# KyleJHarper/tyche

Measured on AMD Instinct MI355X. Metric: GiB/s device-resident LZ4 compress+decompress, 1M×16KiB pages, 1/2/4/8 GPU, higher is better.
Workload: dtype u8

## Files before the change

### tyche_amd/csrc/lz4_decode_lc.hip

```cpp
#include <hip/hip_runtime.h>

#include "engine.h"
#include "lane_ring.h"
#include "lds_io.h"
#include "lds_qword.h"

namespace tyche {

#if defined(TYCHE_ABLATE) && TYCHE_ABLATE
#define LC_ABLATE(bit) ((TYCHE_ABLATE & (bit)) != 0)
#else
#define LC_ABLATE(bit) false
#endif

#ifdef TYCHE_PROFILE
__device__ unsigned long long g_lcprof[16];
#define LPROF_DECL                                  \
    unsigned long long _pt = clock64(), _acc[16]; \
    for (int _k = 0; _k < 16; _k++) _acc[_k] = 0;
#define LPROF_MARK(k)                  \
    do {                               \
        unsigned long long _n = clock64(); \
        _acc[k] += _n - _pt;           \
        _pt = _n;                      \
    } while (0)
#define LPROF_ADD(k, v) do { _acc[k] += (unsigned long long)(v); } while (0)
#define LPROF_END                                                              \
    do {                                                                       \
        if (lane == 0)                                                         \
            for (int _k = 0; _k < 16; _k++) atomicAdd(&g_lcprof[_k], _acc[_k]); \
    } while (0)
#else
#define LPROF_DECL
#define LPROF_MARK(k) do { } while (0)
#define LPROF_ADD(k, v) do { } while (0)
#define LPROF_END do { } while (0)
#endif

namespace {

__device__ __forceinline__ void lc_lut_load(const uint32_t *lut, int32_t c, uint32_t *ent) {
    const uint8_t *p = (const uint8_t *)lut + 48 * c;
    const uint64_t a = lq(p), b = lq(p + 8), x = lq(p + 16), y = lq(p + 24);
    ent[0] = (uint32_t)a;
    ent[1] = (uint32_t)(a >> 32);
    ent[2] = (uint32_t)b;
    ent[3] = (uint32_t)(b >> 32);
    ent[4] = (uint32_t)x;
    ent[5] = (uint32_t)(x >> 32);
    ent[6] = (uint32_t)y;
    ent[7] = (uint32_t)(y >> 32);
    ent[8] = ld32(p + 32);
}

#include "lz4_lc_core.h"

template <int32_t R>
struct LCL {
    static_assert(lc_ring_ok<R>(), "ring too small for the flush granule (lc_budget)");
    static constexpr uint32_t win = 0;
    static constexpr uint32_t ring = 64u * kLWS;
    static constexpr uint32_t tab_out = ring + 64u * (uint32_t)R;
    static constexpr uint32_t tab_fl = tab_out + 64u * 8u;
    static constexpr int32_t max_pieces = (lc_budget<R>() + kLcLine - 1) / 16 + 1;
    static constexpr uint32_t own = tab_fl + 64u * 4u;
    static constexpr uint32_t lut = own + ((64u * (uint32_t)max_pieces * 2u + 15u) & ~15u);
    static constexpr uint32_t total = lut + (uint32_t)kLutBytes;
};

struct LMeta {
    const uint8_t *in;
    uint8_t *out;
    uint32_t L, C;
};
__device__ __forceinline__ LMeta lmeta(const tyche_batch_t &b, size_t idx) {
    const PageRef r = batch_page(b, idx);
    return LMeta{r.src, r.dst, r.src_len, r.dst_cap};
}

struct LWin {
    u128 c0, c1, c2, c3;
    uint32_t sh;
};
__device__ __forceinline__ LWin wload(const uint8_t *__restrict__ in, int32_t ns, int32_t L) {
    LWin w;
    if (L >= 16) {
        const int32_t top = L - 16;
        const int32_t a0 = min(ns, top), a1 = min(ns + 16, top), a2 = min(ns + 32, top), a3 = min(ns + 48, top);
        w.c0 = ld16(in + a0);
        w.c1 = ld16(in + a1);
        w.c2 = ld16(in + a2);
        w.c3 = ld16(in + a3);
        w.sh = (uint32_t)min(ns - a0, 16) | ((uint32_t)min(ns + 16 - a1, 16) << 8) |
               ((uint32_t)min(ns + 32 - a2, 16) << 16) | ((uint32_t)min(ns + 48 - a3, 16) << 24);
    } else {
        w.c0 = chunk16z(in, ns, L);
        w.c1 = chunk16z(in, ns + 16, L);
        w.c2 = chunk16z(in, ns + 32, L);
        w.c3 = chunk16z(in, ns + 48, L);
        w.sh = 0;
    }
    return w;
}
__device__ __forceinline__ u128 wshift(u128 v, uint32_t k) {
    k &= 0xFFu;
    return k >= 16u ? (u128)0 : (k == 0u ? v : v >> (8u * k));
}
__device__ __forceinline__ void lc_put_piece(uint8_t *base, int32_t k, u128 v) {
    lq(LC_Q(base, k), (uint64_t)v);
    lq(LC_Q(base, k + 1), (uint64_t)(v >> 64));
}
__device__ __forceinline__ u128 lc_get_piece(const uint8_t *base, int32_t k) {
    return (u128)lq(LC_Q(base, k)) | ((u128)lq(LC_Q(base, k + 1)) << 64);
}
__device__ __forceinline__ void wstore(uint8_t *w16, const LWin &w) {
    if (w.sh == 0) {
        lc_put_piece(w16, 0, w.c0);
        lc_put_piece(w16, 2, w.c1);
        lc_put_piece(w16, 4, w.c2);
        lc_put_piece(w16, 6, w.c3);
    } else {
        lc_put_piece(w16, 0, wshift(w.c0, w.sh));
        lc_put_piece(w16, 2, wshift(w.c1, w.sh >> 8));
        lc_put_piece(w16, 4, wshift(w.c2, w.sh >> 16));
        lc_put_piece(w16, 6, wshift(w.c3, w.sh >> 24));
    }
}

constexpr int kVmDrain = 0x0F70;

__device__ bool lpage_start(const tyche_batch_t &b, uint32_t in_cap, uint32_t out_cap, size_t idx, size_t G,
                            LPage &P, uint8_t *w16) {
    for (; idx < b.count; idx += G) {
        const LMeta m = lmeta(b, idx);
        int32_t rv;
        if (m.L > in_cap || m.C > out_cap) {
            rv = kResultTooLarge;
        } else if (m.C == 0) {
            rv = (m.L == 1 && ld1(m.in) == 0) ? 0 : -1;
        } else if (m.L == 0) {
            rv = -1;
        } else {
            P.in = m.in;
            P.out = m.out;
            P.L = (int32_t)m.L;
            P.C = (int32_t)m.C;
            P.idx = idx;
            P.ip = P.op = P.fl = P.wb = 0;
            P.tail = 0;
            P.lp = P.lrem = P.moff = P.mrem = P.mtok = P.hdr = P.term = 0;
            wstore(w16, wload(P.in, 0, P.L));
            __builtin_amdgcn_s_waitcnt(kVmDrain);
            return true;
        }
        b.results[idx] = rv;
    }
    return false;
}

__device__ __attribute__((aligned(64))) uint8_t g_lc_pad[64];

template <int32_t N>
__device__ __forceinline__ void far_load(const LPage &P, bool far, int32_t src, uint32_t rec, u32x4 (&fv)[N], int32_t t) {
    if (LC_ABLATE(1024)) far = false;
    if (far) {
        const uint8_t *a = P.out + src;
        asm volatile("global_load_dwordx4 %0, %1, off" : "+v"(fv[kFarPer * t]) : "v"(a) : "memory");
        if (kFarPer == 2 && ((rec >> 10) & 63u) > 16u)
            asm volatile("global_load_dwordx4 %0, %1, off offset:16" : "+v"(fv[kFarPer * t + (kFarPer - 1)]) : "v"(a) : "memory");
    }
}
template <int32_t N>
__device__ __forceinline__ void lc_far_wait(u32x4 (&fv)[N]) {
    asm volatile("s_waitcnt vmcnt(4)" ::: "memory");
#pragma unroll
    for (int32_t i = 0; i < N; i++) asm volatile("" : "+v"(fv[i]));
}

#ifndef LC_WPE
#define LC_WPE 2
#endif
template <int32_t R>
__global__ __launch_bounds__(64) __attribute__((amdgpu_waves_per_eu(LC_WPE))) void lz4_decode_lc_kernel(tyche_batch_t b, uint32_t in_cap, uint32_t out_cap) {
    typedef LCL<R> Lay;
    extern __shared__ __attribute__((aligned(16))) uint8_t smem[];
    const uint32_t lane = threadIdx.x;
    uint8_t *ring = smem + Lay::ring + lane * 8u;
    uint8_t *w16 = smem + Lay::win + lane * 8u;
    uint64_t *tab_out = (uint64_t *)(smem + Lay::tab_out);
    uint32_t *tab_fl = (uint32_t *)(smem + Lay::tab_fl);
    uint16_t *own = (uint16_t *)(smem + Lay::own);
    const uint32_t *lut = (const uint32_t *)(smem + Lay::lut);
    const size_t G = (size_t)gridDim.x * 64u;
    if (lane <= 16) {
        uint32_t ent[kLutStride];
        lc_lut_entry((int32_t)lane, ent);
        for (int32_t j = 0; j < kLutStride; j++) ld32(smem + Lay::lut + 48u * lane + 4u * (uint32_t)j, ent[j]);
    }

    LPage P;
    bool live = lpage_start(b, in_cap, out_cap, (size_t)blockIdx.x * 64u + lane, G, P, w16);
    LPROF_DECL
    while (__builtin_amdgcn_ballot_w64(live) != 0) {
        LPROF_ADD(0, 1);
        LPROF_MARK(9);
        const int32_t op0 = P.op;
        int32_t st = live ? kLParse : kLCut, rv = 0, nrec = 0;
        uint32_t rec[kLC + 1];
        u32x4 fv[kFarPer * (kLC + 1)];
#pragma unroll
        for (int32_t i = 0; i < kFarPer * (kLC + 1); i++) fv[i] = u32x4{0u, 0u, 0u, 0u};
        bool go = live, gen = false;
        int32_t need_gen = 0;
        uint64_t wq[4];
        lc_wread(w16, lc_x0(P), wq);
        bool far0 = false, far1 = false;
        int32_t src0 = 0, src1 = 0;
#pragma unroll
        for (int32_t t = 0; t < kLC; t++) {
            rec[t] = 0;
            bool far = false;
            int32_t src = 0;
            if (go) {
                const int32_t k = parse_fast<R>(P, w16, op0, rec[t], far, src, wq);
                if (k == 1) {
                    nrec = t + 1;
                } else {
                    go = false;
                    need_gen = (k == 2 || t == 0) ? 1 : 0;
                    if (k == 0 && t != 0) st = kLCut;
                }
            }
            if (t == 0) {
                far0 = far;
                src0 = src;
            } else if (t == 1) {
                far1 = far;
                src1 = src;
                LPROF_MARK(1);
                __builtin_amdgcn_s_waitcnt(kVmDrain);
                LPROF_MARK(2);
                asm volatile("" ::: "memory");
                far_load(P, far0, src0, rec[0], fv, 0);
                far_load(P, far1, src1, rec[1], fv, 1);
            } else {
                far_load(P, far, src, rec[t], fv, t);
            }
        }
        LPROF_MARK(3);
        rec[kLC] = 0;
        {
            bool far = false;
            int32_t src = 0;
            if (__builtin_amdgcn_ballot_w64(need_gen != 0) != 0 && need_gen)
                gen = parse_slot<R>(P, w16, op0, false, st, rv, rec[kLC], far, src);
            const bool deep = need_gen && !gen && nrec == 0 && st == kLCut;
            if (__builtin_amdgcn_ballot_w64(deep) != 0 && deep) {
                st = kLParse;
                gen = parse_slot<R>(P, w16, op0, true, st, rv, rec[kLC], far, src);
            }
            far_load(P, far && gen, src, rec[kLC], fv, kLC);
        }
        LPROF_MARK(4);
        LPROF_ADD(12, __builtin_amdgcn_ballot_w64(need_gen != 0) != 0);
        const bool ended = live && st == kLEnd;
        const int32_t nwb = (P.lrem > 0 ? P.lp : P.ip) & ~15;
        const bool wlive = live && !ended;
        const LWin nw = wload(wlive ? P.in : g_lc_pad, wlive ? nwb : 0, wlive ? P.L : 64);
        if (ended && rv < 0) {
            nrec = 0;
            gen = false;
        }

        LPROF_MARK(5);
        lc_far_wait(fv);
        if (LC_ABLATE(8192)) {
            const LWin xw = wload(wlive ? P.in : g_lc_pad, wlive ? min(nwb + 64, max(P.L - 64, 0)) : 0, wlive ? P.L : 64);
            __builtin_amdgcn_s_waitcnt(kVmDrain);
            if (xw.c0 == (u128)0x123457 && xw.c3 == (u128)1) P.tail ^= 1;
        }
        if (live && !LC_ABLATE(4096)) {
            u128 farv[kFarPer * (kLC + 1)];
#pragma unroll
            for (int32_t i = 0; i < kFarPer * (kLC + 1); i++) farv[i] = __builtin_bit_cast(u128, fv[i]);
            uint64_t tail = P.tail;
            copy_records<R>(ring, w16, op0, tail, rec, farv, nrec, gen, lut);
            P.tail = tail;
        }
        LPROF_MARK(6);

        if (live && !ended) {
            P.wb = nwb;
            wstore(w16, nw);
        }
        LPROF_MARK(7);
        const int32_t lend = !live ? 0 : (ended && rv < 0) ? P.fl : (P.op & ~(kLcLine - 1));
        const int32_t nl = live ? (lend - P.fl) >> 4 : 0;
        const int32_t incl = wave_incl_sum(nl);
        const int32_t total = (int32_t)rdlane((uint32_t)incl, 63);
        if (total > 0) {
            constexpr int32_t MP = Lay::max_pieces;
            tab_out[lane] = (uint64_t)(uintptr_t)P.out;
            tab_fl[lane] = (uint32_t)P.fl;
#pragma unroll
            for (int32_t k = 0; k < MP; k++)
                if (k < nl) own[incl - nl + k] = (uint16_t)(lane | ((uint32_t)k << 6));
            asm volatile("" ::: "memory");
            const int32_t iters = (total + 63) >> 6;
            uint32_t e[MP];
#pragma unroll
            for (int32_t it = 0; it < MP; it++) e[it] = it < iters ? (uint32_t)own[lane + 64 * it] : 0u;
            uint64_t o[MP];
            int32_t f[MP];
#pragma unroll
            for (int32_t it = 0; it < MP; it++) {
                o[it] = 0;
                f[it] = 0;
                if (it < iters) {
                    const uint32_t L2 = e[it] & 63u;
                    o[it] = tab_out[L2];
                    f[it] = (int32_t)tab_fl[L2] + 16 * (int32_t)(e[it] >> 6);
                }
            }
            u128 v[MP];
#pragma unroll
            for (int32_t it = 0; it < MP; it++)
                v[it] = it < iters ? lc_get_piece(smem + Lay::ring + (e[it] & 63u) * 8u, lc_row<R>(f[it] >> 3))
                                   : (u128)0;
#pragma unroll
            for (int32_t it = 0; it < MP; it++) {
                if ((int32_t)lane + 64 * it < total) {
                    uint8_t *dst = (uint8_t *)(uintptr_t)o[it] + f[it];
                    if (!LC_ABLATE(2048)) st16f(dst, v[it]);
                    else if (v[it] == (u128)0x1234567) dst[0] = 1;
                }
            }
            asm volatile("" ::: "memory");
        }
        if (live) P.fl = lend > P.fl ? lend : P.fl;
        LPROF_MARK(8);
        LPROF_ADD(13, total);
        LPROF_ADD(14, __builtin_popcountll(__builtin_amdgcn_ballot_w64(ended)));

        if (ended) {
            if (rv >= 0) {
                for (int32_t a = P.fl; a < P.op; a += 16) {
                    const u128 v = lc_get_piece(ring, lc_row<R>(a >> 3));
                    if (a + 16 <= P.op) {
                        st16(P.out + a, v);
                    } else {
                        for (int32_t x = a; x < P.op; x++) st1(P.out + x, (uint32_t)(v >> (8 * (x - a))) & 0xFFu);
                    }
                }
            }
            b.results[P.idx] = rv;
            live = lpage_start(b, in_cap, out_cap, P.idx + G, G, P, w16);
        }
        LPROF_MARK(10);
        asm volatile("" ::: "memory");
    }
    LPROF_END;
}

}

#ifdef TYCHE_PROFILE
extern "C" int tyche_debug_lc_profile(unsigned long long *host16, int reset) {
    if (reset) {
        unsigned long long z[16] = {0};
        return hipMemcpyToSymbol(HIP_SYMBOL(g_lcprof), z, sizeof(z)) == hipSuccess ? 0 : 1;
    }
    return hipMemcpyFromSymbol(host16, HIP_SYMBOL(g_lcprof), sizeof(unsigned long long) * 16) == hipSuccess ? 0 : 1;
}
#endif

hipError_t launch_lz4_decode_lc(const tyche_batch_t &b, uint32_t in_cap, uint32_t out_cap, hipStream_t s) {
    if (b.count == 0) return hipSuccess;
    const long r = knob("LZ4_LC_RING", 192);
#if LC_LINE == 16
    const void *k = r == 256   ? (const void *)lz4_decode_lc_kernel<256>
                    : r == 192 ? (const void *)lz4_decode_lc_kernel<192>
                    : r == 160 ? (const void *)lz4_decode_lc_kernel<160>
                               : (const void *)lz4_decode_lc_kernel<128>;
    const size_t lds = r == 256   ? LCL<256>::total
                       : r == 192 ? LCL<192>::total
                       : r == 160 ? LCL<160>::total
                                  : LCL<128>::total;
#else
    const void *k = r == 256 ? (const void *)lz4_decode_lc_kernel<256> : (const void *)lz4_decode_lc_kernel<192>;
    const size_t lds = r == 256 ? LCL<256>::total : LCL<192>::total;
#endif
    const size_t ncu = prepare_launch(k);
    size_t waves = blocks_per_cu(k, 64, lds);
    const long env_waves = knob("LZ4_LC_WAVES", 8);
    if (env_waves > 0) waves = std::min<size_t>(waves, (size_t)env_waves);
    const size_t grid = std::min<size_t>((b.count + 63) / 64, ncu * waves);
    void *args[] = {(void *)&b, &in_cap, &out_cap};
    (void)hipLaunchKernel(k, dim3((unsigned)grid), dim3(64), args, lds, s);
    return hipGetLastError();
}

}
```

### tyche_amd/csrc/lz4_lc_core.h

```cpp
#pragma once

#ifndef LC_FN
#define LC_FN __device__ __forceinline__
#endif
#ifndef LC_RCP
#define LC_RCP(x) __builtin_amdgcn_rcpf(x)
#endif
#ifndef LC_BARRIER
#define LC_BARRIER() asm volatile("" ::: "memory")
#endif
#ifndef LC_Q
#define LC_Q(base, k) ((base) + ((uint32_t)(k) << 9))
#endif
#ifndef LC_PERM
#define LC_PERM(hi, lo, sel) __builtin_amdgcn_perm((hi), (lo), (sel))
#endif
#ifndef LC_UMUL24
#define LC_UMUL24(a, b) __umul24((a), (b))
#define LC_MUL24(a, b) __mul24((a), (b))
#endif

constexpr int32_t kLutStride = 12;
constexpr int32_t kLutBytes = 17 * kLutStride * 4;
LC_FN void lc_lut_entry(int32_t c, uint32_t *ent) {
// ... 82 lines not shown
    lq(LC_Q(ring, r1), o1);
    lq(LC_Q(ring, r2), o2);
    const uint32_t k = (s + (uint32_t)n) >> 3;
    return k == 0 ? o0 : (k == 1 ? o1 : o2);
}

struct LPage {
    const uint8_t *in;
    uint8_t *out;
    int32_t L, C;
    size_t idx;
    int32_t ip;
    int32_t op;
    int32_t fl;
    int32_t wb;
    uint64_t tail;
    int32_t lp, lrem;
    int32_t moff, mrem;
    int32_t mtok;
    int32_t hdr, term;
};

enum : int32_t { kLParse = 0, kLCut = 1, kLEnd = 2 };

#ifndef LC_LINE
#define LC_LINE 16
#endif
constexpr int32_t kLcLine = LC_LINE;
static_assert(kLcLine == 16 || kLcLine == 64, "flush granule");
template <int32_t R>
constexpr int32_t lc_near() { return R - 24; }
template <int32_t R>
constexpr int32_t lc_budget() { return R - 24 - kLcLine; }
template <int32_t R>
constexpr bool lc_ring_ok() { return lc_budget<R>() >= 47; }

LC_FN uint32_t lc_rec(int32_t lpr, int32_t n1, int32_t n2, int32_t off) {
    return (uint32_t)lpr | ((uint32_t)n1 << 6) | ((uint32_t)n2 << 10) | ((uint32_t)off << 16);
}

LC_FN uint64_t win8(uint64_t q0, uint64_t q1, uint64_t q2, uint64_t q3, uint32_t r) {
    const uint32_t k = r >> 3;
    const uint64_t a = k == 0 ? q0 : (k == 1 ? q1 : q2), b = k == 0 ? q1 : (k == 1 ? q2 : q3);
    return funnel8(a, b, r & 7u);
}

LC_FN void lc_wread(const uint8_t *w16, int32_t x, uint64_t (&q)[4]) {
    const int32_t k = x >> 3;
    q[0] = lq(LC_Q(w16, k));
    q[1] = lq(LC_Q(w16, k + 1));
    q[2] = lq(LC_Q(w16, k + 2));
    q[3] = lq(LC_Q(w16, k + 3));
}
LC_FN int32_t lc_x0(const LPage &P) {
    return (P.lrem == 0 && P.mrem == 0 && P.hdr == 0) ? min(P.ip - P.wb, kLW) : 0;
}

template <int32_t R>
LC_FN int32_t parse_fast(LPage &P, const uint8_t *w16, int32_t op0, uint32_t &rec, bool &far, int32_t &src,
                         uint64_t (&q)[4]) {
    const int32_t room = op0 + lc_budget<R>() - P.op;
    const bool isA = (P.mrem != 0) & (P.lrem == 0);
    const int32_t nA = min(P.mrem, 32);
    const int32_t nB = min(min(P.lrem, 15), P.wb + kLW - P.lp);
    const bool isB = (P.lrem != 0) & (nB < P.lrem);
    const bool fresh = (P.lrem == 0) & (P.mrem == 0) & (P.hdr == 0);
    const int32_t x = fresh ? P.ip - P.wb : 0;
    const uint64_t q0 = q[0], q1 = q[1], q2 = q[2], q3 = q[3];
    const uint32_t s = (uint32_t)x & 7u;
    const uint32_t token = (uint32_t)(win8(q0, q1, q2, q3, s) & 0xFFu);
    const int32_t lit = (int32_t)(token >> 4), mn = (int32_t)(token & 15u);
    const int32_t need = 1 + lit + (mn == 15 ? 3 : 2);
    lc_wread(w16, min(fresh ? x + need : P.ip - P.wb, kLW), q);
    const uint64_t h = win8(q0, q1, q2, q3, s + 1u + (uint32_t)(lit & 15));
    const int32_t off = (int32_t)(h & 0xFFFFu), ext = (int32_t)((h >> 16) & 0xFFu);
    const int32_t ml = mn == 15 ? 19 + ext : mn + kMinMatch;
    const bool fitC = x + need <= kLW;
    const bool okC = (lit != 15) & !((mn == 15) & (ext == 255)) &
                     (P.op + lit <= P.C - kMfLimit) & (P.ip + 1 + lit <= P.L - 8) &
                     (off <= P.op + lit) &
                     !((mn == 15) & (P.ip + need > P.L - kLastLiterals)) &
                     (P.op + lit + ml <= P.C - kLastLiterals) &
                     (ml <= 32);
    const int32_t moff = isA ? P.moff : off;
    const int32_t n1 = isA ? 0 : (isB ? nB : lit);
    const int32_t n2f = isA ? nA : (isB ? 0 : ml);
    const int32_t n2 = (LC_FAR16 && moff > lc_near<R>()) ? min(n2f, 16) : n2f;
    const bool fits = n1 + n2 <= room;
    const bool cont = isA | isB;
    const bool stop = !cont & (((P.lrem != 0) & (nB <= 0)) | (fresh & !fitC));
    const bool fast = cont | (fresh & okC);
    const int32_t k = stop ? 0 : (fast ? (fits ? 1 : 0) : 2);
    const bool emit = (k == 1);
    far = emit & (n2 > 0) & (moff > lc_near<R>());
    src = emit ? P.op + n1 - moff : src;
    rec = emit ? lc_rec(n1 > 0 ? (isB ? P.lp - P.wb : x + 1) : 0, n1, n2, moff) : rec;
    P.op += emit ? n1 + n2 : 0;
    P.mrem -= (emit & isA) ? n2 : 0;
    P.lp += (emit & isB) ? n1 : 0;
    P.lrem -= (emit & isB) ? n1 : 0;
    P.ip += (emit & fresh) ? need : 0;
    if (LC_FAR16) {
        P.mrem += (emit & fresh) ? ml - n2 : 0;
        P.moff = (emit & fresh) ? off : P.moff;
    }
    return k;
}


LC_FN uint32_t lbyte(const LPage &P, const uint8_t *w16, int32_t p, bool deep, bool &miss) {
    if (p < P.wb + kLW) {
        const int32_t i = p - P.wb;
        return lb(LC_Q(w16, i >> 3) + (i & 7));
    }
    if (deep) return sbyte(P.in, p, P.L);
    miss = true;
    return 0;
}

template <int32_t R>
LC_FN bool parse_slot(LPage &P, const uint8_t *w16, int32_t op0, bool deep, int32_t &st,
                                           int32_t &rv, uint32_t &rec, bool &far, int32_t &src) {
    constexpr int32_t kBudget = lc_budget<R>();
    const int32_t wend = P.wb + kLW;
    bool miss = false;
    if (P.lrem == 0 && P.mrem == 0 && P.hdr == 0) {
        const int32_t ip = P.ip;
        const uint32_t token = lbyte(P, w16, ip, deep, miss);
        int32_t lit = (int32_t)(token >> 4), pos = 1;
        if (lit == kRunMask) {
            uint32_t s;
            do {
                s = lbyte(P, w16, ip + pos, deep, miss);
                pos++;
                lit += (int32_t)s;
            } while (!miss && ip + pos < P.L - kRunMask && s == 255);
        }
        if (miss) {
            st = kLCut;
            return false;
        }
        const bool last = P.op + lit > P.C - kMfLimit || ip + pos + lit > P.L - 8;
        if (last && (ip + pos + lit != P.L || P.op + lit > P.C)) {
            rv = -(ip + pos) - 1;
            st = kLEnd;
            return false;
        }
        P.term = last ? 1 : 0;
        P.hdr = last ? 0 : 1;
        P.mtok = (int32_t)(token & 15u);
        P.lp = ip + pos;
        P.lrem = lit;
        P.ip = ip + pos + lit;
    }
    int32_t n1 = min(P.lrem, 15);
    n1 = min(n1, wend - P.lp);
    if (n1 < 0) n1 = 0;
    if (P.lrem > 0 && n1 == 0) {
// ... 115 lines not shown
```

### tyche_amd/_build.py

```python
from __future__ import annotations

import concurrent.futures as cf
import os
import subprocess

HERE = os.path.dirname(os.path.abspath(__file__))
CSRC = os.path.join(HERE, "csrc")
BUILD = os.path.join(HERE, "..", "build", "tyche_amd")
LIB = os.path.join(HERE, "libtyche_codec.so")
SOURCES = ["engine.hip", "lz4_decode.hip", "lz4_decode_lane.hip", "lz4_decode_lc.hip", "lz4_encode.hip", "lz4_encode_exact.hip", "lz4_encode_hc.hip", "lz4_encode_large.hip", "lz4_decode_large.hip", "lz4_encode_dict.hip", "lz4_decode_dict.hip", "lz4_dict_train.hip", "zlib_inflate.hip", "zstd_decode.hip", "zstd_encode.hip", "zlib_deflate.hip", "pagegen.hip", "pack.hip", "host_batch.hip",
           "errno_guard.hip"]
HIPCC = os.environ.get("HIPCC", "/opt/rocm/bin/hipcc")
ARCH = "gfx950"
FLAGS = ["--offload-arch=" + ARCH, "-O3", "-fPIC", "-std=c++17", "-Wall", "-Wno-unused-variable",
         "-munsafe-fp-atomics", "-I" + os.path.join(HERE, "..", "include")]
LEGACY_SOURCES = ["legacy/lz4_decode_lane_legacy.hip", "legacy/lz4_decode_quad.hip"]
NO_LSV = ["-mllvm", "-amdgpu-load-store-vectorizer=false"]
SOURCE_FLAGS = {"lz4_encode.hip": NO_LSV, "lz4_encode_dict.hip": NO_LSV, "zstd_encode.hip": NO_LSV, "zlib_deflate.hip": NO_LSV, "zstd_decode.hip": NO_LSV}


def kernel_sources_digest() -> str:
    import hashlib
    h = hashlib.sha256()
    files = sorted(f for f in os.listdir(CSRC) if f.endswith((".hip", ".h")))
    for f in files:
        h.update(f.encode())
        h.update(open(os.path.join(CSRC, f), "rb").read())
    h.update(open(os.path.join(HERE, "..", "include", "tyche_codec.h"), "rb").read())
    return h.hexdigest()[:16]


def _newer(target: str, deps: list[str]) -> bool:
    if not os.path.exists(target):
        return False
    t = os.path.getmtime(target)
    return all(os.path.getmtime(d) <= t for d in deps)


def build(force: bool = False, verbose: bool = False, profile: bool = False, ablate: int = 0,
          eablate: int = 0, defines: tuple = (), legacy: bool = False) -> str:
    if legacy:
        defines = tuple(defines) + ("TYCHE_LEGACY_DECODERS",)
    tag = ("_prof" if profile else "") + (f"_abl{ablate}" if ablate else "") + (f"_eabl{eablate}" if eablate else "") + \
        "".join("_" + d.replace("TYCHE_", "").replace("=", "").lower() for d in defines)
    build_dir = BUILD + tag
    lib_path = LIB.replace(".so", tag + ".so")
    flags = FLAGS + (["-DTYCHE_PROFILE"] if profile else []) + ([f"-DTYCHE_ABLATE={ablate}"] if ablate else []) + \
        ([f"-DTYCHE_EABLATE={eablate}"] if eablate else []) + ["-D" + d for d in defines]
    os.makedirs(build_dir, exist_ok=True)
    headers = [os.path.join(CSRC, f) for f in os.listdir(CSRC) if f.endswith(".h")]
    headers.append(os.path.join(HERE, "..", "include", "tyche_codec.h"))
    objs = []
    jobs = []
    sources = SOURCES[:-1] + (LEGACY_SOURCES if legacy else []) + SOURCES[-1:]
    for src in sources:
        s = os.path.join(CSRC, src)
        o = os.path.join(build_dir, src.replace("/", "_").replace(".hip", ".o"))
        objs.append(o)
        if force or not _newer(o, [s] + headers):
            jobs.append([HIPCC] + flags + SOURCE_FLAGS.get(src, []) + ["-c", s, "-o", o])

    def run(cmd):
        if verbose:
# ... 38 lines not shown
```

### tyche_amd/csrc/engine.h

```cpp
#pragma once
#include <hip/hip_runtime.h>

#include <algorithm>
#include <stdint.h>

#include "../../include/tyche_codec.h"

namespace tyche {

constexpr int32_t kResultTooLarge = INT32_MIN;

constexpr int kMinMatch = 4;
constexpr int kLastLiterals = 5;
constexpr int kMfLimit = 12;
constexpr int kRunMask = 15;

__host__ __device__ inline uint32_t lz4_bound(uint32_t n) {
    return n > 0x7E000000u ? 0u : n + n / 255u + 16u;
}

struct PageRef {
    const uint8_t *src;
    uint32_t src_len;
    uint8_t *dst;
    uint32_t dst_cap;
};

template <typename T>
__device__ __forceinline__ T ld_meta(const T *p, size_t i) {
    return ((const __attribute__((address_space(4))) T *)(uintptr_t)p)[i];
}

__device__ inline PageRef batch_page(const tyche_batch_t &b, size_t i) {
    PageRef r;
    uint64_t so = b.src_offsets ? ld_meta(b.src_offsets, i) : (uint64_t)i * b.src_stride;
    uint64_t dof = b.dst_offsets ? ld_meta(b.dst_offsets, i) : (uint64_t)i * b.dst_stride;
    r.src = (const uint8_t *)b.src + so;
    r.src_len = b.src_lengths ? ld_meta(b.src_lengths, i) : b.src_length;
    r.dst = (uint8_t *)b.dst + dof;
    r.dst_cap = b.dst_capacities ? ld_meta(b.dst_capacities, i) : b.dst_capacity;
    return r;
}

#define WAVE_SYNC() __builtin_amdgcn_wave_barrier()

size_t blocks_per_cu(const void *kernel, uint32_t threads, size_t lds);
size_t page_grid(const void *kernel, uint32_t threads, size_t lds, size_t count, const char *cap_knob = nullptr);

hipError_t launch_lz4_decode(const tyche_batch_t &b, uint32_t in_cap, uint32_t out_cap, hipStream_t s,
                             bool allow_lane = true);
bool lz4_lane_decode_wanted(size_t count, uint32_t in_cap, uint32_t out_cap);
hipError_t launch_lz4_decode_lane(const tyche_batch_t &b, uint32_t in_cap, uint32_t out_cap, hipStream_t s);
hipError_t launch_lz4_decode_quad(const tyche_batch_t &b, uint32_t in_cap, uint32_t out_cap, hipStream_t s);
hipError_t launch_lz4_decode_lc(const tyche_batch_t &b, uint32_t in_cap, uint32_t out_cap, hipStream_t s);
hipError_t launch_lz4_encode(const tyche_batch_t &b, uint32_t in_cap, hipStream_t s);
hipError_t launch_lz4_encode_exact(const tyche_batch_t &b, uint32_t in_cap, hipStream_t s);
hipError_t launch_lz4_encode_hc(const tyche_batch_t &b, uint32_t in_cap, hipStream_t s);
hipError_t launch_lz4_encode_large(const tyche_batch_t &b, uint32_t in_cap, uint32_t min_len, hipStream_t s);
hipError_t launch_lz4_decode_large(const tyche_batch_t &b, uint32_t in_cap, uint32_t out_cap, hipStream_t s);
struct Lz4DictDev {
    const uint8_t *dec;
    const uint16_t *table;
    const uint8_t *enc;
    uint32_t dlen, dpad, enc_len, enc_stride;
};
hipError_t launch_lz4_encode_dict(const tyche_batch_t &b, uint32_t in_cap, const Lz4DictDev &d, bool per_page,
                                  hipStream_t s);
hipError_t launch_lz4_decode_dict(const tyche_batch_t &b, uint32_t in_cap, uint32_t out_cap, const Lz4DictDev &d,
                                  bool per_page, hipStream_t s);
struct TrainResult {
    uint32_t dict_len = 0;
    bool too_long = false;
    uint64_t total_bytes = 0;
    const char *step = "";
};
hipError_t train_lz4_dict(const tyche_batch_t &b, uint32_t in_cap, uint32_t dict_len, hipStream_t s, uint8_t *dict_out,
                          TrainResult *res);
hipError_t launch_pack(const tyche_pack_t &p, hipStream_t s, const char **step);
uint64_t pack_plan_host(size_t n, const int32_t *results, uint32_t max_length, uint32_t align, uint64_t capacity,
                        uint64_t state[2], uint64_t *offsets, uint32_t *lengths);
hipError_t launch_zstd_encode(const tyche_batch_t &b, uint32_t in_cap, hipStream_t s);
hipError_t launch_zlib_deflate(const tyche_batch_t &b, uint32_t in_cap, hipStream_t s);
hipError_t launch_zlib_inflate(const tyche_batch_t &b, uint32_t out_cap, hipStream_t s);
hipError_t launch_zstd_decode(const tyche_batch_t &b, uint32_t in_cap, uint32_t out_cap, hipStream_t s);
size_t zstd_dict_seed_bytes();
void zstd_dict_seed_table(const uint8_t *tail, uint32_t n, void *table_out);
hipError_t launch_zstd_encode_dict(const tyche_batch_t &b, uint32_t in_cap, const Lz4DictDev &d, const void *seed,
                                   bool per_page, hipStream_t s);
hipError_t launch_zstd_decode_dict(const tyche_batch_t &b, uint32_t in_cap, uint32_t out_cap, const Lz4DictDev &d,
                                   bool per_page, hipStream_t s);
class WorkCounter {
  public:
    explicit WorkCounter(hipStream_t s, bool claims = true);
    ~WorkCounter();
    WorkCounter(const WorkCounter &) = delete;
    WorkCounter &operator=(const WorkCounter &) = delete;
    unsigned *get() const { return p_; }

  private:
    hipStream_t s_;
    int dev_ = -1, idx_ = -1;
    unsigned *p_ = nullptr;
};
class ScratchLease {
  public:
    ScratchLease(hipStream_t s, size_t bytes);
    ~ScratchLease();
// ... 23 lines not shown
```

Measured before the change: 191.5.

## Widen LZ4 fast-parse path and alias flush tables over window rows

Result: no change. 192.8, median of 6 (+0.7%).

```diff
diff --git a/tyche_amd/csrc/lz4_decode_lc.hip b/tyche_amd/csrc/lz4_decode_lc.hip
--- a/tyche_amd/csrc/lz4_decode_lc.hip
+++ b/tyche_amd/csrc/lz4_decode_lc.hip
@@ -55,16 +55,23 @@
 
 #include "lz4_lc_core.h"
 
+#ifndef LC_ALIAS
+#define LC_ALIAS 1
+#endif
+
 template <int32_t R>
 struct LCL {
     static_assert(lc_ring_ok<R>(), "ring too small for the flush granule (lc_budget)");
     static constexpr uint32_t win = 0;
     static constexpr uint32_t ring = 64u * kLWS;
-    static constexpr uint32_t tab_out = ring + 64u * (uint32_t)R;
+    static constexpr uint32_t ring_end = ring + 64u * (uint32_t)R;
+    static constexpr uint32_t tab_out = LC_ALIAS ? win : ring_end;
     static constexpr uint32_t tab_fl = tab_out + 64u * 8u;
     static constexpr int32_t max_pieces = (lc_budget<R>() + kLcLine - 1) / 16 + 1;
     static constexpr uint32_t own = tab_fl + 64u * 4u;
-    static constexpr uint32_t lut = own + ((64u * (uint32_t)max_pieces * 2u + 15u) & ~15u);
+    static constexpr uint32_t tab_end = own + ((64u * (uint32_t)max_pieces * 2u + 15u) & ~15u);
+    static_assert(!LC_ALIAS || tab_end <= ring, "the flush tables must fit the window rows they lie over");
+    static constexpr uint32_t lut = LC_ALIAS ? ring_end : tab_end;
     static constexpr uint32_t total = lut + (uint32_t)kLutBytes;
 };
 
@@ -289,10 +296,23 @@
         }
         LPROF_MARK(6);
 
+#if LC_ALIAS
+        u128 np0 = nw.c0, np1 = nw.c1, np2 = nw.c2, np3 = nw.c3;
+        if (nw.sh != 0) {
+            np0 = wshift(np0, nw.sh);
+            np1 = wshift(np1, nw.sh >> 8);
+            np2 = wshift(np2, nw.sh >> 16);
+            np3 = wshift(np3, nw.sh >> 24);
+        }
+        u32x4 nq0 = __builtin_bit_cast(u32x4, np0), nq1 = __builtin_bit_cast(u32x4, np1),
+              nq2 = __builtin_bit_cast(u32x4, np2), nq3 = __builtin_bit_cast(u32x4, np3);
+        asm volatile("" : "+v"(nq0), "+v"(nq1), "+v"(nq2), "+v"(nq3));
+#else
         if (live && !ended) {
             P.wb = nwb;
             wstore(w16, nw);
         }
+#endif
         LPROF_MARK(7);
         const int32_t lend = !live ? 0 : (ended && rv < 0) ? P.fl : (P.op & ~(kLcLine - 1));
         const int32_t nl = live ? (lend - P.fl) >> 4 : 0;
@@ -338,6 +358,16 @@
             asm volatile("" ::: "memory");
         }
         if (live) P.fl = lend > P.fl ? lend : P.fl;
+#if LC_ALIAS
+        asm volatile("" : "+v"(nq0), "+v"(nq1), "+v"(nq2), "+v"(nq3));
+        if (live && !ended) {
+            P.wb = nwb;
+            lc_put_piece(w16, 0, __builtin_bit_cast(u128, nq0));
+            lc_put_piece(w16, 2, __builtin_bit_cast(u128, nq1));
+            lc_put_piece(w16, 4, __builtin_bit_cast(u128, nq2));
+            lc_put_piece(w16, 6, __builtin_bit_cast(u128, nq3));
+        }
+#endif
         LPROF_MARK(8);
         LPROF_ADD(13, total);
         LPROF_ADD(14, __builtin_popcountll(__builtin_amdgcn_ballot_w64(ended)));
diff --git a/tyche_amd/csrc/lz4_lc_core.h b/tyche_amd/csrc/lz4_lc_core.h
--- a/tyche_amd/csrc/lz4_lc_core.h
+++ b/tyche_amd/csrc/lz4_lc_core.h
@@ -158,58 +158,78 @@
     q[2] = lq(LC_Q(w16, k + 2));
     q[3] = lq(LC_Q(w16, k + 3));
 }
-LC_FN int32_t lc_x0(const LPage &P) {
-    return (P.lrem == 0 && P.mrem == 0 && P.hdr == 0) ? min(P.ip - P.wb, kLW) : 0;
-}
+LC_FN int32_t lc_x0(const LPage &P) { return min(P.ip - P.wb, kLW); }
+
+#ifndef LC_STAT
+#define LC_STAT(i, c) do { } while (0)
+#endif
+
+#ifndef LC_FASTX
+#define LC_FASTX 1
+#endif
+constexpr bool kFxM = (LC_FASTX & 1) != 0, kFxL = (LC_FASTX & 2) != 0, kFxH = (LC_FASTX & 4) != 0;
 
 template <int32_t R>
 LC_FN int32_t parse_fast(LPage &P, const uint8_t *w16, int32_t op0, uint32_t &rec, bool &far, int32_t &src,
                          uint64_t (&q)[4]) {
     const int32_t room = op0 + lc_budget<R>() - P.op;
-    const bool isA = (P.mrem != 0) & (P.lrem == 0);
-    const int32_t nA = min(P.mrem, 32);
+    const bool inrun = P.lrem != 0;
+    const bool isA = (P.mrem != 0) & !inrun;
     const int32_t nB = min(min(P.lrem, 15), P.wb + kLW - P.lp);
-    const bool isB = (P.lrem != 0) & (nB < P.lrem);
-    const bool fresh = (P.lrem == 0) & (P.mrem == 0) & (P.hdr == 0);
-    const int32_t x = fresh ? P.ip - P.wb : 0;
+    const bool isB = inrun & (nB < P.lrem) & (nB > 0);
+    const bool isH = kFxH & (P.hdr != 0) & (nB == P.lrem);
+    const bool fresh = !inrun & (P.mrem == 0) & (P.hdr == 0);
+    const int32_t x = P.ip - P.wb;
     const uint64_t q0 = q[0], q1 = q[1], q2 = q[2], q3 = q[3];
     const uint32_t s = (uint32_t)x & 7u;
-    const uint32_t token = (uint32_t)(win8(q0, q1, q2, q3, s) & 0xFFu);
-    const int32_t lit = (int32_t)(token >> 4), mn = (int32_t)(token & 15u);
-    const int32_t need = 1 + lit + (mn == 15 ? 3 : 2);
-    lc_wread(w16, min(fresh ? x + need : P.ip - P.wb, kLW), q);
-    const uint64_t h = win8(q0, q1, q2, q3, s + 1u + (uint32_t)(lit & 15));
+    const uint64_t w0 = win8(q0, q1, q2, q3, s);
+    const uint32_t token = (uint32_t)w0 & 0xFFu;
+    const int32_t lit4 = (int32_t)(token >> 4), lext = (int32_t)((uint32_t)(w0 >> 8) & 0xFFu);
+    const bool isL = kFxL & fresh & (lit4 == 15);
+    const int32_t lit = (kFxL && lit4 == 15) ? 15 + lext : lit4;
+    const int32_t mn = (kFxH && !fresh) ? P.mtok : (int32_t)(token & 15u);
+    const int32_t hl = mn == 15 ? 3 : 2;
+    const int32_t need = fresh ? (isL ? 2 + lit : 1 + lit4 + hl) : (isH ? hl : 0);
+    lc_wread(w16, min(x + need, kLW), q);
+    const uint64_t h = win8(q0, q1, q2, q3, (kFxH && !fresh) ? s : s + 1u + (uint32_t)lit4);
     const int32_t off = (int32_t)(h & 0xFFFFu), ext = (int32_t)((h >> 16) & 0xFFu);
     const int32_t ml = mn == 15 ? 19 + ext : mn + kMinMatch;
-    const bool fitC = x + need <= kLW;
-    const bool okC = (lit != 15) & !((mn == 15) & (ext == 255)) &
-                     (P.op + lit <= P.C - kMfLimit) & (P.ip + 1 + lit <= P.L - 8) &
-                     (off <= P.op + lit) &
-                     !((mn == 15) & (P.ip + need > P.L - kLastLiterals)) &
-                     (P.op + lit + ml <= P.C - kLastLiterals) &
-                     (ml <= 32);
+    const int32_t nH = isH ? nB : lit4;
+    const bool okHdr = !((mn == 15) & (ext == 255)) &
+                       (off <= P.op + nH) &
+                       !((mn == 15) & (P.ip + need > P.L - kLastLiterals)) &
+                       (P.op + nH + ml <= P.C - kLastLiterals);
+    const bool notLast = (P.op + lit <= P.C - kMfLimit) & (P.ip + (isL ? 2 : 1) + lit <= P.L - 8);
+    const bool okC = (lit4 != 15) & notLast & okHdr & (kFxM | (ml <= 32));
+    const bool okL = (lext != 255) & notLast;
+    const int32_t nL = min(15, kLW - (x + 2));
+    const bool fit = isL ? nL > 0 : x + need <= kLW;
+    const bool hasM = isA | isH | (fresh & !isL);
     const int32_t moff = isA ? P.moff : off;
-    const int32_t n1 = isA ? 0 : (isB ? nB : lit);
-    const int32_t n2f = isA ? nA : (isB ? 0 : ml);
+    const int32_t n1 = isA ? 0 : (inrun ? nB : (isL ? nL : (fresh ? lit4 : 0)));
+    const int32_t n2f = hasM ? min(isA ? P.mrem : ml, 32) : 0;
     const int32_t n2 = (LC_FAR16 && moff > lc_near<R>()) ? min(n2f, 16) : n2f;
     const bool fits = n1 + n2 <= room;
     const bool cont = isA | isB;
-    const bool stop = !cont & (((P.lrem != 0) & (nB <= 0)) | (fresh & !fitC));
-    const bool fast = cont | (fresh & okC);
+    const bool stop = (inrun & (nB <= 0)) | (fresh & !fit);
+    const bool fast = cont | (fresh & (isL ? okL : okC)) | (isH & fit & okHdr);
     const int32_t k = stop ? 0 : (fast ? (fits ? 1 : 0) : 2);
     const bool emit = (k == 1);
+    LC_STAT(0, emit & fresh & !isL & (ml > 32));
+    LC_STAT(1, emit & isL);
+    LC_STAT(2, emit & isH);
     far = emit & (n2 > 0) & (moff > lc_near<R>());
     src = emit ? P.op + n1 - moff : src;
-    rec = emit ? lc_rec(n1 > 0 ? (isB ? P.lp - P.wb : x + 1) : 0, n1, n2, moff) : rec;
+    rec = emit ? lc_rec(n1 > 0 ? (inrun ? P.lp - P.wb : x + (isL ? 2 : 1)) : 0, n1, n2, moff) : rec;
     P.op += emit ? n1 + n2 : 0;
-    P.mrem -= (emit & isA) ? n2 : 0;
-    P.lp += (emit & isB) ? n1 : 0;
-    P.lrem -= (emit & isB) ? n1 : 0;
-    P.ip += (emit & fresh) ? need : 0;
-    if (LC_FAR16) {
-        P.mrem += (emit & fresh) ? ml - n2 : 0;
-        P.moff = (emit & fresh) ? off : P.moff;
-    }
+    P.lp = (emit & isL) ? P.ip + 2 + n1 : P.lp + ((emit & inrun) ? n1 : 0);
+    P.lrem = (emit & isL) ? lit - n1 : P.lrem - ((emit & inrun) ? n1 : 0);
+    P.mtok = (emit & isL) ? mn : P.mtok;
+    P.hdr = (emit & isL) ? 1 : ((emit & isH) ? 0 : P.hdr);
+    P.ip += emit ? need : 0;
+    const bool newM = emit & hasM & !isA;
+    P.mrem = newM ? ml - n2 : P.mrem - ((emit & isA) ? n2 : 0);
+    P.moff = newM ? off : P.moff;
     return k;
 }
 
```

## Order LZ4 decode pages by compressed length for lane load balance

Applied to the files above, without the earlier changes.

Result: faster. 191.0 before, 193.3 after, median of 6 (+1.2%).

```diff
diff --git a/tyche_amd/_build.py b/tyche_amd/_build.py
--- a/tyche_amd/_build.py
+++ b/tyche_amd/_build.py
@@ -8,7 +8,7 @@
 CSRC = os.path.join(HERE, "csrc")
 BUILD = os.path.join(HERE, "..", "build", "tyche_amd")
 LIB = os.path.join(HERE, "libtyche_codec.so")
-SOURCES = ["engine.hip", "lz4_decode.hip", "lz4_decode_lane.hip", "lz4_decode_lc.hip", "lz4_encode.hip", "lz4_encode_exact.hip", "lz4_encode_hc.hip", "lz4_encode_large.hip", "lz4_decode_large.hip", "lz4_encode_dict.hip", "lz4_decode_dict.hip", "lz4_dict_train.hip", "zlib_inflate.hip", "zstd_decode.hip", "zstd_encode.hip", "zlib_deflate.hip", "pagegen.hip", "pack.hip", "host_batch.hip",
+SOURCES = ["engine.hip", "lz4_decode.hip", "lz4_decode_lane.hip", "lz4_decode_lc.hip", "lz4_encode.hip", "lz4_encode_exact.hip", "lz4_encode_hc.hip", "lz4_encode_large.hip", "lz4_decode_large.hip", "lz4_encode_dict.hip", "lz4_decode_dict.hip", "lz4_dict_train.hip", "zlib_inflate.hip", "zstd_decode.hip", "zstd_encode.hip", "zlib_deflate.hip", "pagegen.hip", "pack.hip", "page_order.hip", "host_batch.hip",
            "errno_guard.hip"]
 HIPCC = os.environ.get("HIPCC", "/opt/rocm/bin/hipcc")
 ARCH = "gfx950"
diff --git a/tyche_amd/csrc/engine.h b/tyche_amd/csrc/engine.h
--- a/tyche_amd/csrc/engine.h
+++ b/tyche_amd/csrc/engine.h
@@ -53,6 +53,10 @@
 hipError_t launch_lz4_decode_lane(const tyche_batch_t &b, uint32_t in_cap, uint32_t out_cap, hipStream_t s);
 hipError_t launch_lz4_decode_quad(const tyche_batch_t &b, uint32_t in_cap, uint32_t out_cap, hipStream_t s);
 hipError_t launch_lz4_decode_lc(const tyche_batch_t &b, uint32_t in_cap, uint32_t out_cap, hipStream_t s);
+bool page_order_fits(size_t count, uint32_t window);
+size_t page_order_work_bytes(size_t count, uint32_t window);
+hipError_t launch_page_order(const uint32_t *lengths, size_t count, uint32_t in_cap, uint32_t window, uint32_t *order, void *work,
+                             hipStream_t s);
 hipError_t launch_lz4_encode(const tyche_batch_t &b, uint32_t in_cap, hipStream_t s);
 hipError_t launch_lz4_encode_exact(const tyche_batch_t &b, uint32_t in_cap, hipStream_t s);
 hipError_t launch_lz4_encode_hc(const tyche_batch_t &b, uint32_t in_cap, hipStream_t s);
diff --git a/tyche_amd/csrc/lz4_decode_lc.hip b/tyche_amd/csrc/lz4_decode_lc.hip
--- a/tyche_amd/csrc/lz4_decode_lc.hip
+++ b/tyche_amd/csrc/lz4_decode_lc.hip
@@ -1,9 +1,14 @@
 #include <hip/hip_runtime.h>
+
+#include <atomic>
 
 #include "engine.h"
 #include "lane_ring.h"
 #include "lds_io.h"
 #include "lds_qword.h"
+
+#define PO_HOST 0
+#include "page_order_core.h"
 
 namespace tyche {
 
@@ -15,6 +20,8 @@
 
 #ifdef TYCHE_PROFILE
 __device__ unsigned long long g_lcprof[16];
+constexpr unsigned kLcProfWaves = 4096;
+__device__ unsigned g_lcwave[kLcProfWaves];
 #define LPROF_DECL                                  \
     unsigned long long _pt = clock64(), _acc[16]; \
     for (int _k = 0; _k < 16; _k++) _acc[_k] = 0;
@@ -27,8 +34,10 @@
 #define LPROF_ADD(k, v) do { _acc[k] += (unsigned long long)(v); } while (0)
 #define LPROF_END                                                              \
     do {                                                                       \
-        if (lane == 0)                                                         \
+        if (lane == 0) {                                                       \
             for (int _k = 0; _k < 16; _k++) atomicAdd(&g_lcprof[_k], _acc[_k]); \
+            if (blockIdx.x < kLcProfWaves) g_lcwave[blockIdx.x] = (unsigned)_acc[0]; \
+        }                                                                      \
     } while (0)
 #else
 #define LPROF_DECL
@@ -129,9 +138,29 @@
 
 constexpr int kVmDrain = 0x0F70;
 
+constexpr uint32_t kNoPage = 0xFFFFFFFFu;
+struct LWalk {
+    const uint32_t *order;
+    uint32_t gen;
+    uint32_t nxt;
+};
+__device__ __forceinline__ uint32_t lwalk_load(const LWalk &W, size_t count, uint32_t lane) {
+    const uint64_t s = po::slot(W.gen, blockIdx.x, lane, gridDim.x, count);
+    return s < count ? W.order[s] : kNoPage;
+}
+
+template <bool kOrdered>
 __device__ bool lpage_start(const tyche_batch_t &b, uint32_t in_cap, uint32_t out_cap, size_t idx, size_t G,
-                            LPage &P, uint8_t *w16) {
-    for (; idx < b.count; idx += G) {
+                            LPage &P, uint8_t *w16, LWalk &W, uint32_t lane) {
+    for (;; idx += G) {
+        if (kOrdered) {
+            idx = W.nxt;
+            if (idx >= b.count) return false;
+            W.gen++;
+            W.nxt = lwalk_load(W, b.count, lane);
+        } else if (idx >= b.count) {
+            return false;
+        }
         const LMeta m = lmeta(b, idx);
         int32_t rv;
         if (m.L > in_cap || m.C > out_cap) {
@@ -155,7 +184,6 @@
         }
         b.results[idx] = rv;
     }
-    return false;
 }
 
 __device__ __attribute__((aligned(64))) uint8_t g_lc_pad[64];
@@ -180,8 +208,9 @@
 #ifndef LC_WPE
 #define LC_WPE 2
 #endif
-template <int32_t R>
-__global__ __launch_bounds__(64) __attribute__((amdgpu_waves_per_eu(LC_WPE))) void lz4_decode_lc_kernel(tyche_batch_t b, uint32_t in_cap, uint32_t out_cap) {
+template <int32_t R, bool kOrdered>
+__global__ __launch_bounds__(64) __attribute__((amdgpu_waves_per_eu(LC_WPE))) void lz4_decode_lc_kernel(tyche_batch_t b, uint32_t in_cap, uint32_t out_cap,
+                                                                                                     const uint32_t *order) {
     typedef LCL<R> Lay;
     extern __shared__ __attribute__((aligned(16))) uint8_t smem[];
     const uint32_t lane = threadIdx.x;
@@ -199,7 +228,9 @@
     }
 
     LPage P;
-    bool live = lpage_start(b, in_cap, out_cap, (size_t)blockIdx.x * 64u + lane, G, P, w16);
+    LWalk W{order, 0u, kNoPage};
+    if (kOrdered) W.nxt = lwalk_load(W, b.count, lane);
+    bool live = lpage_start<kOrdered>(b, in_cap, out_cap, (size_t)blockIdx.x * 64u + lane, G, P, w16, W, lane);
     LPROF_DECL
     while (__builtin_amdgcn_ballot_w64(live) != 0) {
         LPROF_ADD(0, 1);
@@ -354,7 +385,7 @@
                 }
             }
             b.results[P.idx] = rv;
-            live = lpage_start(b, in_cap, out_cap, P.idx + G, G, P, w16);
+            live = lpage_start<kOrdered>(b, in_cap, out_cap, P.idx + G, G, P, w16, W, lane);
         }
         LPROF_MARK(10);
         asm volatile("" ::: "memory");
@@ -372,32 +403,64 @@
     }
     return hipMemcpyFromSymbol(host16, HIP_SYMBOL(g_lcprof), sizeof(unsigned long long) * 16) == hipSuccess ? 0 : 1;
 }
+extern "C" int tyche_debug_lc_wave_iters(unsigned *host, int n) {
+    if (n < 0 || (unsigned)n > tyche::kLcProfWaves) return 1;
+    return hipMemcpyFromSymbol(host, HIP_SYMBOL(g_lcwave), sizeof(unsigned) * (size_t)n) == hipSuccess ? 0 : 1;
+}
 #endif
+
+static std::atomic<unsigned long long> g_lc_ordered_launches{0};
+extern "C" unsigned long long tyche_debug_lz4_lc_ordered_launches(void) { return g_lc_ordered_launches.load(); }
+
+constexpr long kLcOrder = 1;
+constexpr long kLcOrderWindow = 4096;
 
 hipError_t launch_lz4_decode_lc(const tyche_batch_t &b, uint32_t in_cap, uint32_t out_cap, hipStream_t s) {
     if (b.count == 0) return hipSuccess;
     const long r = knob("LZ4_LC_RING", 192);
 #if LC_LINE == 16
-    const void *k = r == 256   ? (const void *)lz4_decode_lc_kernel<256>
-                    : r == 192 ? (const void *)lz4_decode_lc_kernel<192>
-                    : r == 160 ? (const void *)lz4_decode_lc_kernel<160>
-                               : (const void *)lz4_decode_lc_kernel<128>;
+#define LC_PICK(ordered)                                                           \
+    (r == 256   ? (const void *)lz4_decode_lc_kernel<256, ordered>                 \
+     : r == 192 ? (const void *)lz4_decode_lc_kernel<192, ordered>                 \
+     : r == 160 ? (const void *)lz4_decode_lc_kernel<160, ordered>                 \
+                : (const void *)lz4_decode_lc_kernel<128, ordered>)
     const size_t lds = r == 256   ? LCL<256>::total
                        : r == 192 ? LCL<192>::total
                        : r == 160 ? LCL<160>::total
                                   : LCL<128>::total;
 #else
-    const void *k = r == 256 ? (const void *)lz4_decode_lc_kernel<256> : (const void *)lz4_decode_lc_kernel<192>;
+#define LC_PICK(ordered) \
+    (r == 256 ? (const void *)lz4_decode_lc_kernel<256, ordered> : (const void *)lz4_decode_lc_kernel<192, ordered>)
     const size_t lds = r == 256 ? LCL<256>::total : LCL<192>::total;
 #endif
+    const void *k = LC_PICK(false);
     const size_t ncu = prepare_launch(k);
     size_t waves = blocks_per_cu(k, 64, lds);
     const long env_waves = knob("LZ4_LC_WAVES", 8);
     if (env_waves > 0) waves = std::min<size_t>(waves, (size_t)env_waves);
-    const size_t grid = std::min<size_t>((b.count + 63) / 64, ncu * waves);
-    void *args[] = {(void *)&b, &in_cap, &out_cap};
+    size_t grid = std::min<size_t>((b.count + 63) / 64, ncu * waves);
+    const long env_grid = knob("LZ4_LC_GRID", 0);
+    if (env_grid > 0) grid = std::min<size_t>(grid, (size_t)env_grid);
+    const long env_window = knob("LZ4_LC_ORDER_WINDOW", kLcOrderWindow);
+    const uint32_t window = env_window > 0 && (unsigned long)env_window < b.count ? (uint32_t)env_window : 0u;
+    const bool ordered = knob("LZ4_LC_ORDER", kLcOrder) != 0 && b.src_lengths && b.count >= 2 * grid * 64 &&
+                         page_order_fits(b.count, window);
+    const size_t order_bytes = (b.count * sizeof(uint32_t) + 255u) & ~(size_t)255u;
+    ScratchLease ws(s, ordered ? order_bytes + page_order_work_bytes(b.count, window) : 0);
+    const uint32_t *order = (const uint32_t *)ws.get();
+    if (ordered) {
+        if (!order) return hipErrorOutOfMemory;
+        const hipError_t e =
+            launch_page_order(b.src_lengths, b.count, in_cap, window, (uint32_t *)ws.get(), (uint8_t *)ws.get() + order_bytes, s);
+        if (e != hipSuccess) return e;
+        k = LC_PICK(true);
+        (void)prepare_launch(k);
+        g_lc_ordered_launches++;
+    }
+    void *args[] = {(void *)&b, &in_cap, &out_cap, &order};
     (void)hipLaunchKernel(k, dim3((unsigned)grid), dim3(64), args, lds, s);
     return hipGetLastError();
-}
-
-}
+#undef LC_PICK
+}
+
+}
diff --git a/tyche_amd/csrc/page_order.hip b/tyche_amd/csrc/page_order.hip
--- /dev/null
+++ b/tyche_amd/csrc/page_order.hip
@@ -0,0 +1,131 @@
+#include <hip/hip_runtime.h>
+
+#include "engine.h"
+
+#define PO_HOST 0
+#include "page_order_core.h"
+
+namespace tyche {
+
+namespace {
+
+constexpr uint32_t kSteps = po::kTile / po::kLanes;
+static_assert(po::kTile % po::kLanes == 0 && po::kBins % po::kLanes == 0, "whole steps of one wave");
+static_assert(po::kBins == 512, "the scatter's ballots cover 9 key bits; the scan runs one thread per key");
+
+__global__ __launch_bounds__(64) void page_order_hist_kernel(const uint32_t *lengths, uint32_t in_cap, uint32_t shift, po::Geo g,
+                                                             uint32_t *hist) {
+    __shared__ uint32_t cnt[po::kBins];
+    const uint32_t lane = threadIdx.x, tile = blockIdx.x;
+    for (uint32_t k = lane; k < po::kBins; k += po::kLanes) cnt[k] = 0;
+    __syncthreads();
+    uint32_t first, end;
+    po::tile_bounds(g, tile, &first, &end);
+#pragma unroll 8
+    for (uint32_t s = 0; s < kSteps; s++) {
+        const uint64_t i = (uint64_t)first + s * po::kLanes + lane;
+        if (i < end) atomicAdd(&cnt[po::rank_key(lengths[i], in_cap, shift)], 1u);
+    }
+    __syncthreads();
+    for (uint32_t k = lane; k < po::kBins; k += po::kLanes) hist[(size_t)tile * po::kBins + k] = cnt[k];
+}
+
+__global__ __launch_bounds__(po::kBins) void page_order_scan_kernel(po::Geo g, uint32_t *hist, uint32_t *base) {
+    __shared__ uint32_t buf[2 * po::kBins];
+    const uint32_t k = threadIdx.x, w = blockIdx.x;
+    uint32_t run = 0;
+    uint32_t *p = hist + (size_t)w * g.tpw * po::kBins + k;
+#pragma unroll 8
+    for (uint32_t j = 0; j < g.tpw; j++) {
+        const uint32_t v = p[(size_t)j * po::kBins];
+        p[(size_t)j * po::kBins] = run;
+        run += v;
+    }
+    uint32_t cur = 0;
+    buf[k] = run;
+    __syncthreads();
+#pragma unroll
+    for (uint32_t d = 1; d < po::kBins; d <<= 1) {
+        const uint32_t x = buf[cur + k] + (k >= d ? buf[cur + k - d] : 0u);
+        cur ^= po::kBins;
+        buf[cur + k] = x;
+        __syncthreads();
+    }
+    base[(size_t)w * po::kBins + k] = buf[cur + k] - run;
+}
+
+__global__ __launch_bounds__(64) void page_order_scatter_kernel(const uint32_t *lengths, uint32_t in_cap, uint32_t shift, po::Geo g,
+                                                                const uint32_t *hist, const uint32_t *base, uint32_t *order) {
+    __shared__ uint32_t cnt[po::kBins];
+    const uint32_t lane = threadIdx.x, tile = blockIdx.x;
+    uint32_t first, end;
+    po::tile_bounds(g, tile, &first, &end);
+    if (first >= end) return;
+    const uint32_t w = tile / g.tpw, w0 = po::window_first(g, w);
+    for (uint32_t k = lane; k < po::kBins; k += po::kLanes)
+        cnt[k] = w0 + base[(size_t)w * po::kBins + k] + hist[(size_t)tile * po::kBins + k];
+    uint32_t key[kSteps];
+#pragma unroll
+    for (uint32_t s = 0; s < kSteps; s++) {
+        const uint64_t i = (uint64_t)first + s * po::kLanes + lane;
+        key[s] = i < end ? po::rank_key(lengths[i], in_cap, shift) : 0u;
+    }
+    __syncthreads();
+    const uint64_t below = ((uint64_t)1 << lane) - 1u;
+#pragma unroll
+    for (uint32_t s = 0; s < kSteps; s++) {
+        const uint64_t i = (uint64_t)first + s * po::kLanes + lane;
+        const bool valid = i < end;
+        if (__ballot(valid) == 0) break;
+        uint64_t peers = __ballot(valid);
+#pragma unroll
+        for (uint32_t bit = 0; bit < 9; bit++) {
+            const bool one = (key[s] >> bit) & 1u;
+            const uint64_t m = __ballot(valid && one);
+            peers &= one ? m : ~m;
+        }
+        const uint32_t at = valid ? cnt[key[s]] : 0u;
+        __syncthreads();
+        if (valid && (peers >> lane) == 1u) cnt[key[s]] = at + (uint32_t)__popcll(peers);
+        __syncthreads();
+        const uint32_t pos = at + (uint32_t)__popcll(peers & below);
+        if (valid && pos < g.count) order[pos] = (uint32_t)i;
+    }
+}
+
+}
+
+bool page_order_fits(size_t count, uint32_t window) {
+    return count > 0 && count <= 0x7FFFFFFFu && po::geometry_ok((uint32_t)count, window);
+}
+
+size_t page_order_work_bytes(size_t count, uint32_t window) {
+    const po::Geo g = po::geometry((uint32_t)count, window);
+    return ((size_t)g.ntiles + g.nwin) * po::kBins * sizeof(uint32_t);
+}
+
+hipError_t launch_page_order(const uint32_t *lengths, size_t count, uint32_t in_cap, uint32_t window, uint32_t *order, void *work,
+                             hipStream_t s) {
+    const po::Geo g = po::geometry((uint32_t)count, window);
+    const uint32_t shift = po::bin_shift(in_cap);
+    uint32_t *hist = (uint32_t *)work, *base = hist + (size_t)g.ntiles * po::kBins;
+    page_order_hist_kernel<<<g.ntiles, 64, 0, s>>>(lengths, in_cap, shift, g, hist);
+    page_order_scan_kernel<<<g.nwin, po::kBins, 0, s>>>(g, hist, base);
+    page_order_scatter_kernel<<<g.ntiles, 64, 0, s>>>(lengths, in_cap, shift, g, hist, base, order);
+    return hipGetLastError();
+}
+
+}
+
+extern "C" int tyche_debug_lz4_page_order(const tyche_batch_t *batch, uint32_t in_cap, uint32_t window, uint32_t *out) {
+    using namespace tyche;
+    if (!batch || !out || !batch->src_lengths || batch->count == 0 || !page_order_fits(batch->count, window)) return 1;
+    const size_t order_bytes = (batch->count * sizeof(uint32_t) + 255u) & ~(size_t)255u;
+    ScratchLease ws(nullptr, order_bytes + page_order_work_bytes(batch->count, window));
+    if (!ws.get()) return 2;
+    uint32_t *order = (uint32_t *)ws.get();
+    if (launch_page_order(batch->src_lengths, batch->count, in_cap, window, order, (uint8_t *)ws.get() + order_bytes, nullptr) !=
+        hipSuccess)
+        return 2;
+    return hipMemcpy(out, order, batch->count * sizeof(uint32_t), hipMemcpyDeviceToHost) == hipSuccess ? 0 : 2;
+}
diff --git a/tyche_amd/csrc/page_order_core.h b/tyche_amd/csrc/page_order_core.h
--- /dev/null
+++ b/tyche_amd/csrc/page_order_core.h
@@ -0,0 +1,68 @@
+#pragma once
+#include <stdint.h>
+
+#if PO_HOST
+#define PO_FN static inline
+#else
+#define PO_FN __host__ __device__ __forceinline__
+#endif
+
+namespace po {
+
+constexpr uint32_t kBins = 512;
+constexpr uint32_t kTile = 2048;
+constexpr uint32_t kLanes = 64;
+
+PO_FN uint32_t bin_shift(uint32_t in_cap) {
+    uint32_t s = 0;
+    while ((in_cap >> s) >= kBins) s++;
+    return s;
+}
+PO_FN uint32_t bin_of(uint32_t length, uint32_t in_cap, uint32_t shift) { return (length < in_cap ? length : in_cap) >> shift; }
+PO_FN uint32_t rank_key(uint32_t length, uint32_t in_cap, uint32_t shift) { return kBins - 1u - bin_of(length, in_cap, shift); }
+
+struct Geo {
+    uint32_t count;
+    uint32_t win;
+    uint32_t nwin;
+    uint32_t tpw;
+    uint32_t ntiles;
+};
+PO_FN Geo geometry(uint32_t count, uint32_t window) {
+    Geo g;
+    g.count = count;
+    g.win = window == 0 || window > count ? count : window;
+    g.nwin = (uint32_t)(((uint64_t)count + g.win - 1u) / g.win);
+    g.tpw = (uint32_t)(((uint64_t)g.win + kTile - 1u) / kTile);
+    g.ntiles = g.nwin * g.tpw;
+    return g;
+}
+PO_FN bool geometry_ok(uint32_t count, uint32_t window) {
+    const uint32_t win = window == 0 || window > count ? count : window;
+    const uint64_t nwin = ((uint64_t)count + win - 1u) / win, tpw = ((uint64_t)win + kTile - 1u) / kTile;
+    return nwin * tpw <= (1u << 20);
+}
+PO_FN uint32_t window_first(const Geo &g, uint32_t w) { return (uint32_t)((uint64_t)w * g.win); }
+PO_FN void tile_bounds(const Geo &g, uint32_t t, uint32_t *first, uint32_t *end) {
+    const uint32_t w = t / g.tpw, j = t % g.tpw;
+    const uint64_t w0 = (uint64_t)w * g.win;
+    uint64_t w1 = w0 + g.win;
+    if (w1 > g.count) w1 = g.count;
+    uint64_t a = w0 + (uint64_t)j * kTile, b = a + kTile;
+    if (a > w1) a = w1;
+    if (b > w1) b = w1;
+    *first = (uint32_t)a;
+    *end = (uint32_t)b;
+}
+
+PO_FN uint64_t slot(uint64_t k, uint32_t wave, uint32_t lane, uint32_t grid, uint64_t count) {
+    const uint64_t G = (uint64_t)grid * kLanes, t = (uint64_t)wave * kLanes + lane;
+    const uint64_t s = k * G + ((k & 1u) ? G - 1u - t : t);
+    return s < count ? s : count;
+}
+PO_FN uint64_t generations(uint32_t grid, uint64_t count) {
+    const uint64_t G = (uint64_t)grid * kLanes;
+    return (count + G - 1u) / G;
+}
+
+}
```
